# solislemuslab/BayesianNetworkRegression.jl

Hardware: AMD Instinct MI355X
Metric: Gibbs iterations/sec (all chains) (higher is better)
Workload: dtype f64; 1 GPU; synthetic n=500 V=100 (q=5050) R=7, 8 chains total, 8 per GPU; chains_total=8, chains_per_gpu=8, seed=20240501

## Files before the change

bayesiannetworkregression.jl_amd/csrc/bnr_kernels.h:

```cpp
#pragma once
#include "bnr_device.h"

#define BNR_RMAX 32
#define BNR_NB 32
#define BNR_GT 64


#define BNR_GLOBAL_PTR(member) d.member = (decltype(d.member))(__attribute__((address_space(1))) void *)(unsigned long long)(d.member)
__device__ __forceinline__ bnr_dev bnr_globalized(const bnr_dev *src)
{
    bnr_dev d = *src;
    BNR_GLOBAL_PTR(X); BNR_GLOBAL_PTR(X8); BNR_GLOBAL_PTR(XM); BNR_GLOBAL_PTR(Sdig); BNR_GLOBAL_PTR(y); BNR_GLOBAL_PTR(ek); BNR_GLOBAL_PTR(el); BNR_GLOBAL_PTR(trace); BNR_GLOBAL_PTR(plan);
    BNR_GLOBAL_PTR(pbase); BNR_GLOBAL_PTR(Wbuf); BNR_GLOBAL_PTR(sz); BNR_GLOBAL_PTR(PW); BNR_GLOBAL_PTR(PA); BNR_GLOBAL_PTR(PG);
    BNR_GLOBAL_PTR(Gpart); BNR_GLOBAL_PTR(E); BNR_GLOBAL_PTR(gmap); BNR_GLOBAL_PTR(a3); BNR_GLOBAL_PTR(xw); BNR_GLOBAL_PTR(a4);
    BNR_GLOBAL_PTR(res); BNR_GLOBAL_PTR(xg); BNR_GLOBAL_PTR(bw); BNR_GLOBAL_PTR(wv); BNR_GLOBAL_PTR(scal); BNR_GLOBAL_PTR(Minv);
    BNR_GLOBAL_PTR(Psum); BNR_GLOBAL_PTR(counters); BNR_GLOBAL_PTR(dbg); BNR_GLOBAL_PTR(stamp); BNR_GLOBAL_PTR(gprog); BNR_GLOBAL_PTR(gmapc); BNR_GLOBAL_PTR(dfctl);
    return d;
}
struct bnr_one {
    bnr_dev d;
    static constexpr bool whole = true, lone = true;
    __device__ __forceinline__ const bnr_dev &get() const { return d; }
    __device__ __forceinline__ const bnr_dev &get_x() const { return d; }
    __device__ __forceinline__ const bnr_dev &at(int) const { return d; }
// ... 902 lines not shown
    unsigned char *sX = (unsigned char *)smem_i8;
    bnr_i4 *sDig = (bnr_i4 *)(sX + 4 * BNR_I8_TB);
    const int tid = threadIdx.x, wave = tid >> 6, lane = tid & 63, ln = lane & 15, lq = lane >> 4;
    const int ng = cd.kcp / 16;
    for (int idx = tid; idx < L * ng; idx += 256) {
        const int l = idx / ng, g = idx % ng;
        sDig[idx] = *(const bnr_i4 *)(cd.Sdig + (size_t)l * cd.kslab + (size_t)ks * cd.kcp + 16 * g);
    }
    const int srow = tid >> 3, scol = tid & 7;
    const unsigned char *gI = cd.XM + (size_t)(ti * BNR_GT + srow) * cd.kslab + (size_t)ks * cd.kcp + 16 * scol;
    const unsigned char *gJ = cd.XM + (size_t)(tj * BNR_GT + srow) * cd.kslab + (size_t)ks * cd.kcp + 16 * scol;
    const size_t r32 = (size_t)32 * cd.kslab;
    const int soff = srow * BNR_I8_RS + 16 * scol;
    bnr_i4 r0 = {0, 0, 0, 0}, r1 = r0, r2 = r0, r3 = r0;
    const int nbatch = cd.kcp / 128, nb = nbatch + ((cd.kcp % 128) ? 1 : 0);
    auto load = [&](int b) {
        const int o = 128 * b;
        if (b < nbatch || scol < 4) { r0 = *(const bnr_i4 *)(gI + o); r1 = *(const bnr_i4 *)(gI + r32 + o); r2 = *(const bnr_i4 *)(gJ + o); r3 = *(const bnr_i4 *)(gJ + r32 + o); }
    };
    auto store = [&](int buf) {
        unsigned char *d = sX + buf * 2 * BNR_I8_TB + soff;
        *(bnr_i4 *)d = r0; *(bnr_i4 *)(d + 32 * BNR_I8_RS) = r1; *(bnr_i4 *)(d + BNR_I8_TB) = r2; *(bnr_i4 *)(d + BNR_I8_TB + 32 * BNR_I8_RS) = r3;
    };
    bnr_i4 acc[L][4];
#pragma unroll
    for (int l = 0; l < L; ++l)
#pragma unroll
        for (int a = 0; a < 4; ++a) acc[l][a] = bnr_i4{0, 0, 0, 0};
    load(0); store(0);
    if (nb > 1) load(1);
    __syncthreads();
    const int fa = ln * BNR_I8_RS + 16 * lq + BNR_I8_TB, fb = (wave * 16 + ln) * BNR_I8_RS + 16 * lq;
    for (int b = 0; b < nb; ++b) {
        const unsigned char *xb = sX + (b & 1) * 2 * BNR_I8_TB;
        const int nk = (b < nbatch) ? 2 : 1;
        bnr_i4 dgall;
        {
            const int pl = ln & 7, pk = ln >> 3, lcl = pl < L ? pl : L - 1;
            int gi = (2 * b + pk) * 4 + lq;
            gi = gi < ng ? gi : ng - 1;
            dgall = sDig[lcl * ng + gi];
        }
#pragma unroll
        for (int kk = 0; kk < 2; ++kk) {
            if (kk >= nk) break;
            const bnr_i4 a0 = *(const bnr_i4 *)(xb + fa + 64 * kk), a1 = *(const bnr_i4 *)(xb + fa + 16 * BNR_I8_RS + 64 * kk);
            const bnr_i4 a2 = *(const bnr_i4 *)(xb + fa + 32 * BNR_I8_RS + 64 * kk), a3 = *(const bnr_i4 *)(xb + fa + 48 * BNR_I8_RS + 64 * kk);
            const bnr_i4 b0 = *(const bnr_i4 *)(xb + fb + 64 * kk);
#pragma unroll
            for (int l = 0; l < L; ++l) {
                bnr_i4 m0;
                if (kk == 0) {
#pragma unroll
                    for (int d = 0; d < 4; ++d) m0[d] = b0[d] & bnr_row_bcast<0>(dgall[d], l);
                } else {
#pragma unroll
                    for (int d = 0; d < 4; ++d) m0[d] = b0[d] & bnr_row_bcast<8>(dgall[d], l);
                }
                acc[l][0] = __builtin_amdgcn_mfma_i32_16x16x64_i8(a0, m0, acc[l][0], 0, 0, 0);
                acc[l][1] = __builtin_amdgcn_mfma_i32_16x16x64_i8(a1, m0, acc[l][1], 0, 0, 0);
                acc[l][2] = __builtin_amdgcn_mfma_i32_16x16x64_i8(a2, m0, acc[l][2], 0, 0, 0);
                acc[l][3] = __builtin_amdgcn_mfma_i32_16x16x64_i8(a3, m0, acc[l][3], 0, 0, 0);
            }
            if (kk == 0 && b + 1 < nb) { store((b + 1) & 1); if (b + 2 < nb) load(b + 2); }
        }
        __syncthreads();
    }
    const double sc = -cd.scal[SC_I8SCALE];
    double *out = cd.Gpart + ((size_t)ks * ntl + t) * (BNR_GT * BNR_GT);
#pragma unroll
    for (int jt = 0; jt < 4; ++jt)
#pragma unroll
        for (int r = 0; r < 4; ++r) {
            double v = (double)acc[0][jt][r];
#pragma unroll
            for (int l = 1; l < L; ++l) v = v * 256.0 + (double)acc[l][jt][r];
            out[(jt * 16 + 4 * lq + r) * BNR_GT + wave * 16 + ln] = v * sc;
        }
}

__host__ __device__ inline int bnr_ldE(int n_pad) { return 2 * n_pad + BNR_NB; }

#define BNR_CRITICAL_PATH() __builtin_amdgcn_s_setprio(3)
template <class SRC>
__global__ __launch_bounds__(256) void k_gram_reduce(const SRC chain_src, int s)
{
    BNR_CRITICAL_PATH();
    const bnr_dev &cd = chain_src.get();
    int t = blockIdx.x, ti = 0;
    while ((ti + 1) * (ti + 2) / 2 <= t) ++ti;
    int tj = t - ti * (ti + 1) / 2;
    const int ntl = cd.ntile * (cd.ntile + 1) / 2;
    const size_t ld = bnr_ldE(cd.n_pad), tsz = BNR_GT * BNR_GT;
    const int idx = blockIdx.y * 512 + 2 * threadIdx.x;
    const double *src = cd.Gpart + (size_t)t * tsz + idx;
    bnr_d2 acc = {0.0, 0.0};
    int ks = 0;
    for (; ks + 3 < cd.ksplit; ks += 4) {
        bnr_d2 v0 = *(const bnr_d2 *)(src + (size_t)ks * ntl * tsz), v1 = *(const bnr_d2 *)(src + (size_t)(ks + 1) * ntl * tsz);
        bnr_d2 v2 = *(const bnr_d2 *)(src + (size_t)(ks + 2) * ntl * tsz), v3 = *(const bnr_d2 *)(src + (size_t)(ks + 3) * ntl * tsz);
        acc += v0; acc += v1; acc += v2; acc += v3;
    }
    for (; ks < cd.ksplit; ++ks) acc += *(const bnr_d2 *)(src + (size_t)ks * ntl * tsz);
    const int i = ti * BNR_GT + idx % BNR_GT, j = tj * BNR_GT + idx / BNR_GT;
    if (i == j) acc[0] += 1.0;
    if (i + 1 == j) acc[1] += 1.0;
    *(bnr_d2 *)(cd.E + (size_t)i + ld * j) = acc;
    const int nwg = gridDim.x * gridDim.y, wg = blockIdx.x * gridDim.y + blockIdx.y, np = cd.n_pad;
    for (size_t e = ((size_t)wg * 256 + threadIdx.x) * 2; e < (size_t)np * np; e += (size_t)nwg * 512) {
        int r = (int)(e % np), c = (int)(e / np);
        if (r / BNR_NB > c / BNR_NB) continue;
        bnr_d2 v = {(r == c) ? 1.0 : 0.0, (r + 1 == c) ? 1.0 : 0.0};
        *(bnr_d2 *)(cd.E + (size_t)(np + r) + ld * c) = v;
    }
    if (threadIdx.x == 0) cd.stamp[blockIdx.x * 8 + blockIdx.y] = cd.plan[cd.pbase[0] + s].it;
    if (blockIdx.x == 0 && blockIdx.y == 0 && (int)threadIdx.x <= cd.ntile) cd.gprog[threadIdx.x] = 0u;
}

__device__ __forceinline__ double bnr_readlane(double v, int srclane)
{
    int lo = __double2loint(v), hi = __double2hiint(v);
    lo = __builtin_amdgcn_readlane(lo, srclane);
    hi = __builtin_amdgcn_readlane(hi, srclane);
    return __hiloint2double(hi, lo);
}
#define BNR_LP (BNR_NB + 1)
__host__ __device__ inline int bnr_chol_npanel(int nbk, int p) { (void)p; return nbk + 1; }
__host__ __device__ inline int bnr_chol_ntile(int nbk, int p)
{
    if (p == 0) return 0;
    int m = nbk - (p + 1);
    return m * (m + 1) / 2 + m * p;
}
__host__ __device__ inline int bnr_chol_nsuper(int nbk, int p)
{
    if (p == 0) return 0;
    int ms = (nbk - (p + 1) + 1) / 2;
    return ms * (ms + 1) / 2 + ms * ((p + 1) / 2);
}

__device__ __forceinline__ bnr_d4 bnr_tile_update(const double *colrows, const double *rowrows, size_t ld, int lane, bnr_d4 c)
{
    const int ln = lane & 15, lk = lane >> 4;
    double av[8], bv[8];
#pragma unroll
    for (int ks = 0; ks < 8; ++ks) {
        av[ks] = colrows[(size_t)ln + ld * (size_t)(4 * ks + lk)];
        bv[ks] = rowrows[(size_t)ln + ld * (size_t)(4 * ks + lk)];
    }
#pragma unroll
    for (int ks = 0; ks < 8; ++ks) c = __builtin_amdgcn_mfma_f64_16x16x4f64(-av[ks], bv[ks], c, 0, 0, 0);
    return c;
}

#define BNR_L1S 80
#define BNR_PIPE_SPINS (1 << 16)
#define BNR_PIPE_SENT_HI 0x7FF8DEAD
__device__ __forceinline__ double bnr_canon_nan(double v) { return v == v ? v : __hiloint2double(0x7FF80000, 0); }
struct alignas(16) bnr_panelp_lds {
    double sD[BNR_NB * BNR_LP], sB[BNR_NB * BNR_LP];
    double sL[BNR_NB][64];
};
__device__ __forceinline__ unsigned bnr_lds_addr(const void *p) { return (unsigned)(unsigned long long)(__attribute__((address_space(3))) const void *)p; }
struct bnr_no_hook { __device__ __forceinline__ void operator()() const {} };
template <int N, int COFF, int PUB, class HOOK = bnr_no_hook>
__device__ __forceinline__ int bnr_sweepN(double (&a)[N], int lane, unsigned pub_addr, HOOK hook = HOOK())
{
    int bad = 0;
    double lprev = 0.0;
    double piv = bnr_readlane(a[0], COFF);
#pragma unroll
    for (int j = 0; j < N; ++j) {
        double tk[N];
        double s1 = 0.0, s2 = 0.0, s3 = 0.0;
        if (j + 1 < N) { s1 = bnr_readlane(a[j + 1], COFF + j + 1); s2 = bnr_readlane(a[j], COFF + j + 1); }
        if (j + 2 < N) s3 = bnr_readlane(a[j], COFF + j + 2);
        if (!(piv > 0.0)) bad = 1;
        double y = __builtin_amdgcn_rsq(piv);
        if (j == 0) hook();
        if (j >= 1) {
#pragma unroll
            for (int k = j + 2; k < N; ++k) tk[k] = bnr_readlane(lprev, COFF + k);
        }
        const double e = fma(-(piv * y), y, 1.0);
        const double rinv = fma(y * e, fma(0.375, e, 0.5), y);
        const double t1 = s2 * rinv;
        piv = fma(-t1, t1, s1);
        double lj = a[j] * rinv;
        a[j] = lj;
        if (PUB == 2) asm volatile("ds_write_b64 %1, %2 offset:%3" : "+v"(piv) : "v"(pub_addr), "v"(lj), "n"(512 * j) : "memory");
        if (j + 1 < N) a[j + 1] = fma(-lj, t1, a[j + 1]);
        if (j + 2 < N) a[j + 2] = fma(-lj, s3 * rinv, a[j + 2]);
        if (j >= 1) {
#pragma unroll
            for (int k = j + 2; k < N; ++k) a[k] = fma(-lprev, tk[k], a[k]);
        }
        lprev = lj;
    }
    return bad;
}
template <int COFF>
__device__ __forceinline__ int bnr_sweep16(double (&a)[16], int lane) { return bnr_sweepN<16, COFF, 0>(a, lane, 0u); }
template <int W>
__device__ __forceinline__ int bnr_pipe_wave(bnr_panelp_lds &sh, int lane, double *dst, size_t ld, unsigned long long *ph = nullptr)
{
#ifdef BNR_STAMPS
#define BNR_PPH(i) do { if (ph && lane == 0) ph[i] = __builtin_amdgcn_s_memtime(); } while (0)
#else
#define BNR_PPH(i) do { } while (0)
#endif
    constexpr int C0 = 8 * W;
    const int rr = lane & 31;
    const double *src = (lane < 32) ? sh.sD : sh.sB;
    double a[8];
#pragma unroll
    for (int c = 0; c < 8; ++c) a[c] = src[rr + BNR_LP * (C0 + c)];
    int bad = 0;
#define BNR_PIPE_HERE(X0, X1) __all(__double2hiint(X0) != BNR_PIPE_SENT_HI && __double2hiint(X1) != BNR_PIPE_SENT_HI)
    unsigned vc = bnr_lds_addr(&sh.sL[0][lane]), vm = bnr_lds_addr(&sh.sL[0][C0 + (lane & 7)]);
    double x0 = 0.0, x1 = 0.0, m0 = 0.0, m1 = 0.0, y0 = 0.0, y1 = 0.0, q0 = 0.0, q1 = 0.0;
#define BNR_DPP_READ4(X0, X1, M0, M1, OFF)                                                                                                                   \
    do { asm volatile("ds_read_b64 %0, %4 offset:%6\n\tds_read_b64 %1, %4 offset:%7\n\tds_read_b64 %2, %5 offset:%6\n\tds_read_b64 %3, %5 offset:%7"          \
                 : "=&v"(X0), "=&v"(X1), "=&v"(M0), "=&v"(M1) : "v"(vc), "v"(vm), "n"(OFF), "n"((OFF) + 512) : "memory");                                    \
         asm volatile("" : "+v"(a[0]), "+v"(a[1]), "+v"(a[2]), "+v"(a[3]), "+v"(a[4]), "+v"(a[5]), "+v"(a[6]), "+v"(a[7])); } while (0)
#define BNR_DPP_WAIT4(X0, X1, M0, M1) asm volatile("s_waitcnt lgkmcnt(0)" : "+v"(X0), "+v"(X1), "+v"(M0), "+v"(M1), "+v"(a[0]), "+v"(a[1]), "+v"(a[2]), "+v"(a[3]), "+v"(a[4]), "+v"(a[5]), "+v"(a[6]), "+v"(a[7]) :: "memory")
#define BNR_DPP_FMA(C, MM, X) asm("v_fmac_f64_dpp %0, -%1, %2 row_newbcast:%3 row_mask:0xf bank_mask:0xf" : "+v"(a[C]) : "v"(MM), "v"(X), "n"(C))
#define BNR_DPP_APPLY(CFROM, X0, X1, M0, M1)                                                                                                                 \
    do { _Pragma("unroll") for (int c_ = (CFROM); c_ < 8; ++c_) {                                                                                            \
             switch (c_) {                                                                                                                                   \
             case 0: BNR_DPP_FMA(0, M0, X0); BNR_DPP_FMA(0, M1, X1); break; case 1: BNR_DPP_FMA(1, M0, X0); BNR_DPP_FMA(1, M1, X1); break;                     \
             case 2: BNR_DPP_FMA(2, M0, X0); BNR_DPP_FMA(2, M1, X1); break; case 3: BNR_DPP_FMA(3, M0, X0); BNR_DPP_FMA(3, M1, X1); break;                     \
             case 4: BNR_DPP_FMA(4, M0, X0); BNR_DPP_FMA(4, M1, X1); break; case 5: BNR_DPP_FMA(5, M0, X0); BNR_DPP_FMA(5, M1, X1); break;                     \
             case 6: BNR_DPP_FMA(6, M0, X0); BNR_DPP_FMA(6, M1, X1); break; default: BNR_DPP_FMA(7, M0, X0); BNR_DPP_FMA(7, M1, X1); break; } } } while (0)
#define BNR_DPP_TRIP(X0, X1, M0, M1, OFF, Y0, Y1, Q0, Q1)                                                                \
    do {                                                                                                                \
        BNR_DPP_WAIT4(X0, X1, M0, M1);                                                                                  \
        if (!BNR_PIPE_HERE(X0, X1)) {                                                                                   \
            int spins = 0;                                                                                              \
            do {                                                                                                        \
                if (++spins > BNR_PIPE_SPINS) { bad = 1; break; }                                                       \
                BNR_DPP_READ4(X0, X1, M0, M1, OFF);                                                                     \
                BNR_DPP_WAIT4(X0, X1, M0, M1);                                                                          \
            } while (!BNR_PIPE_HERE(X0, X1));                                                                           \
        }                                                                                                               \
        BNR_DPP_READ4(Y0, Y1, Q0, Q1, (OFF) + 1024);                                                                    \
        BNR_DPP_APPLY(0, X0, X1, M0, M1);                                                                               \
    } while (0)
    if (W > 0) {
        constexpr int NT = C0 / 2;
        BNR_DPP_READ4(x0, x1, m0, m1, 0);
#pragma unroll 1
        for (int t = 0; t + 2 < NT; t += 2) {
            BNR_DPP_TRIP(x0, x1, m0, m1, 0, y0, y1, q0, q1);
            BNR_DPP_TRIP(y0, y1, q0, q1, 1024, x0, x1, m0, m1);
            vc += 2048; vm += 2048;
        }
        BNR_DPP_TRIP(x0, x1, m0, m1, 0, y0, y1, q0, q1);
        BNR_DPP_WAIT4(y0, y1, q0, q1);
        if (!BNR_PIPE_HERE(y0, y1)) {
            int spins = 0;
            do {
                if (++spins > BNR_PIPE_SPINS) { bad = 1; break; }
                BNR_DPP_READ4(y0, y1, q0, q1, 1024);
                BNR_DPP_WAIT4(y0, y1, q0, q1);
            } while (!BNR_PIPE_HERE(y0, y1));
        }
        BNR_DPP_FMA(0, q0, y0); BNR_DPP_FMA(0, q1, y1); BNR_DPP_FMA(1, q0, y0); BNR_DPP_FMA(1, q1, y1);
    }
    if (W == 1) BNR_PPH(3);
    if (W == 3) BNR_PPH(6);
    bad |= bnr_sweepN<8, C0, (W < 3 ? 2 : 0)>(a, lane, bnr_lds_addr(&sh.sL[C0][lane]), [&]() { if (W > 0) BNR_DPP_APPLY(2, y0, y1, q0, q1); });
    if (W == 0) BNR_PPH(2);
    if (W == 1) BNR_PPH(4);
    if (W == 2) BNR_PPH(5);
    if (W == 3) BNR_PPH(7);
    if (dst && lane >= 32) {
#pragma unroll
        for (int c = 0; c < 8; ++c) dst[(size_t)rr + ld * (size_t)(C0 + c)] = a[c];
    }
    return bad;
}
__device__ __forceinline__ int bnr_panel_sweep_pipe(bnr_panelp_lds &sh, const bnr_d4 &cD, const bnr_d4 &cB, int tid, double *dst, size_t ld, unsigned long long *ph = nullptr)
{
    const int wave = tid >> 6, lane = tid & 63, mt = wave >> 1, nt = wave & 1, ln = lane & 15, lq = lane >> 4;
#ifdef BNR_STAMPS
    if (ph && tid == 0) ph[0] = __builtin_amdgcn_s_memtime();
#endif
    {
        const double sent = __hiloint2double(BNR_PIPE_SENT_HI, 0);
        double *sl = &sh.sL[0][0];
#pragma unroll
        for (int i = 0; i < 6; ++i) sl[tid + 256 * i] = sent;
    }
#pragma unroll
    for (int r = 0; r < 4; ++r) {
        sh.sD[(nt * 16 + ln) + BNR_LP * (mt * 16 + lq + 4 * r)] = bnr_canon_nan(cD[r]);
        sh.sB[(nt * 16 + ln) + BNR_LP * (mt * 16 + lq + 4 * r)] = bnr_canon_nan(cB[r]);
    }
    __syncthreads();
#ifdef BNR_STAMPS
    if (ph && tid == 0) ph[1] = __builtin_amdgcn_s_memtime();
#endif
    if (wave == 0) return bnr_pipe_wave<0>(sh, lane, dst, ld, ph);
    if (wave == 1) return bnr_pipe_wave<1>(sh, lane, dst, ld, ph);
    if (wave == 2) return bnr_pipe_wave<2>(sh, lane, dst, ld, ph);
    return bnr_pipe_wave<3>(sh, lane, dst, ld, ph);
}
template <int NT>
__device__ __forceinline__ void bnr_gsum_frag(const bnr_dev &cd, int rho, int c, int at0, int bt0, int ln, int lq, bnr_d4 (&out)[NT][NT])
{
    const int ti = rho >> 1, tj = c >> 1, ntl = cd.ntile * (cd.ntile + 1) / 2;
    const size_t tsz = BNR_GT * BNR_GT, plane = (size_t)ntl * tsz;
    const double *src = cd.Gpart + (size_t)(ti * (ti + 1) / 2 + tj) * tsz + (size_t)((c & 1) * BNR_NB + 16 * at0 + lq) * BNR_GT + (rho & 1) * BNR_NB + 16 * bt0 + ln;
#pragma unroll
    for (int at = 0; at < NT; ++at)
#pragma unroll
        for (int bt = 0; bt < NT; ++bt) out[at][bt] = bnr_d4{0.0, 0.0, 0.0, 0.0};
    constexpr int KU = NT == 1 ? 8 : 4;
    const int klast = cd.ksplit - 1;
    for (int ks0 = 0; ks0 < cd.ksplit; ks0 += KU) {
        bnr_d4 v[KU][NT][NT];
#pragma unroll
        for (int u = 0; u < KU; ++u) {
            const size_t po = (size_t)(ks0 + u < klast ? ks0 + u : klast) * plane;
#pragma unroll
            for (int at = 0; at < NT; ++at)
#pragma unroll
                for (int bt = 0; bt < NT; ++bt)
#pragma unroll
                    for (int r = 0; r < 4; ++r) v[u][at][bt][r] = *(src + po + (size_t)(16 * at + 4 * r) * BNR_GT + 16 * bt);
        }
#pragma unroll
        for (int u = 0; u < KU; ++u) {
#pragma unroll
            for (int at = 0; at < NT; ++at)
#pragma unroll
                for (int bt = 0; bt < NT; ++bt)
#pragma unroll
                    for (int r = 0; r < 4; ++r) out[at][bt][r] += (ks0 + u <= klast) ? v[u][at][bt][r] : 0.0;
        }
    }
    if (rho == c) {
#pragma unroll
        for (int at = 0; at < NT; ++at)
#pragma unroll
            for (int bt = 0; bt < NT; ++bt)
#pragma unroll
                for (int r = 0; r < 4; ++r) if (16 * (bt0 + bt) + ln == 16 * (at0 + at) + lq + 4 * r) out[at][bt][r] += 1.0;
    }
}
template <int EPW>
__device__ __forceinline__ void bnr_reduce_parts(const bnr_dev &cd, int g0, int nwg, int wg, int s)
{
    constexpr int KB = EPW == 4 ? 4 : 8;
    const int tid = threadIdx.x, t = g0 >> 3, part0 = g0 & 7;
    const int ntl = cd.ntile * (cd.ntile + 1) / 2, ksplit = cd.ksplit;
    const size_t ld = (size_t)2 * cd.n_pad + BNR_NB, tsz = BNR_GT * BNR_GT, plane = (size_t)ntl * tsz;
    const double *src = cd.Gpart + (size_t)t * tsz + part0 * 512 + 2 * tid;
    bnr_d2 v[KB][EPW], acc[EPW];
    const int pb = *(const volatile int *)cd.pbase;
#define BNR_RP_LOAD(KS0)                                                                                                          \
    _Pragma("unroll") for (int u = 0; u < KB; ++u) {                                                                              \
        _Pragma("unroll") for (int e = 0; e < EPW; ++e) v[u][e] = bnr_d2{0.0, 0.0};                                               \
        if ((KS0) + u < ksplit) {                                                                                                 \
            _Pragma("unroll") for (int e = 0; e < EPW; ++e) v[u][e] = *(const bnr_d2 *)(src + (size_t)((KS0) + u) * plane + e * 512); \
        }                                                                                                                         \
    }
    BNR_RP_LOAD(0)
    const unsigned int it = cd.plan[pb + s].it;
    const int np = cd.n_pad;
    for (size_t e = ((size_t)wg * 256 + tid) * 2; e < (size_t)np * np; e += (size_t)nwg * 512) {
        const int r = (int)(e % np), c = (int)(e / np);
        if ((r < BNR_NB && c < BNR_NB) || r / BNR_NB > c / BNR_NB) continue;
        bnr_d2 y = {(r == c) ? 1.0 : 0.0, (r + 1 == c) ? 1.0 : 0.0};
        *(bnr_d2 *)(cd.E + (size_t)(np + r) + ld * c) = y;
    }
    if (wg == 0 && tid <= cd.ntile) cd.gprog[tid] = 0u;
#pragma unroll
    for (int e = 0; e < EPW; ++e) acc[e] = bnr_d2{0.0, 0.0};
    for (int ks0 = 0;;) {
#pragma unroll
        for (int u = 0; u < KB; ++u)
            if (ks0 + u < ksplit) {
#pragma unroll
                for (int e = 0; e < EPW; ++e) acc[e] += v[u][e];
            }
        ks0 += KB;
        if (ks0 >= ksplit) break;
        BNR_RP_LOAD(ks0)
    }
#undef BNR_RP_LOAD
    int ti = 0;
    while ((ti + 1) * (ti + 2) / 2 <= t) ++ti;
    const int tj = t - ti * (ti + 1) / 2;
#pragma unroll
    for (int e = 0; e < EPW; ++e) {
        const int idx = (part0 + e) * 512 + 2 * tid;
        const int i = ti * BNR_GT + idx % BNR_GT, j = tj * BNR_GT + idx / BNR_GT;
        if (i == j) acc[e][0] += 1.0;
        if (i + 1 == j) acc[e][1] += 1.0;
        if (j >= BNR_NB) *(bnr_d2 *)(cd.E + (size_t)i + ld * j) = acc[e];
    }
    if (tid < EPW) cd.stamp[g0 + tid] = it;
#ifdef BNR_STAMPS
    if (tid == 0) atomicMax((unsigned long long *)&cd.dbg[7], (unsigned long long)__builtin_amdgcn_s_memrealtime());
#endif
}
#define BNR_CHOL_WG_PER_CU 4
template <class SRC>
__global__ __launch_bounds__(256, BNR_CHOL_WG_PER_CU) void k_chol_step(const SRC chain_src, int p, int s, int tpw, int spw, int fuse0)
{
    BNR_CRITICAL_PATH();
#ifdef BNR_STAMPS
    const unsigned long long t_entry = __builtin_amdgcn_s_memtime();
#endif
    const bnr_dev &cd = chain_src.get_x();
    __shared__ bnr_panelp_lds sh;
    static_assert(sizeof(sh.sL) == 2 * BNR_NB * BNR_NB * sizeof(double), "the two fetched blocks of panel p - 1 live where the sweep's published columns will be");
    static_assert(BNR_CHOL_WG_PER_CU * sizeof(bnr_panelp_lds) <= 160 * 1024, "BNR_CHOL_WG_PER_CU workgroups must fit a CU's LDS");
    double (*sPO)[BNR_NB * BNR_NB] = (double (*)[BNR_NB * BNR_NB])&sh.sL[0][0];
    const int tid = threadIdx.x, wave = tid >> 6, lane = tid & 63, nbk = cd.n_pad / BNR_NB;
    const size_t ld = bnr_ldE(cd.n_pad);
    const int npanel = bnr_chol_npanel(nbk, p);
    const int pc = p * BNR_NB, kc = pc - BNR_NB;
    const int mt = wave >> 1, nt = wave & 1;
    const int ln = lane & 15, lq = lane >> 4;
    double *E = cd.E;
    if (SRC::whole && p == 0 && (int)blockIdx.y >= npanel) {
        const int wg = (int)blockIdx.y - npanel, nwg = (int)gridDim.y - npanel;
        if (SRC::lone || tpw == 1) bnr_reduce_parts<1>(cd, wg, nwg, wg, s);
        else if (tpw == 4) bnr_reduce_parts<4>(cd, 4 * wg, nwg, wg, s);
        else bnr_reduce_parts<2>(cd, 2 * wg, nwg, wg, s);
        return;
    }
    if ((int)blockIdx.y >= npanel) {
        const int m = nbk - (p + 1);
        if (tpw == 0) {
            const int ms = (m + 1) / 2, ntri = ms * (ms + 1) / 2, nsup = bnr_chol_nsuper(nbk, p);
            for (int u = 0; u < spw; ++u) {
                int t = ((int)blockIdx.y - npanel) * spw + u, R0, C0;
                if (t >= nsup) break;
                bool ident = false;
                if (t < ntri) {
                    int ti = 0;
                    while ((ti + 1) * (ti + 2) / 2 <= t) ++ti;
                    int tj = t - ti * (ti + 1) / 2;
                    R0 = p + 1 + 2 * ti; C0 = p + 1 + 2 * tj;
                } else {
                    t -= ntri;
                    const int ps = (p + 1) / 2;
                    C0 = p + 1 + 2 * (t / ps); R0 = nbk + 2 * (t % ps);
                    ident = true;
                }
                const int rho = R0 + (wave >> 1), j = C0 + (wave & 1);
                const bool ok = j < nbk && (ident ? (rho - nbk < p) : (rho < nbk && rho >= j));
                if (!ok) continue;
                double *cp = E + (size_t)(rho * BNR_NB + ln) + ld * (size_t)(j * BNR_NB + lq);
                bnr_d4 c[2][2];
#pragma unroll
                for (int a = 0; a < 2; ++a)
#pragma unroll
                    for (int b = 0; b < 2; ++b)
#pragma unroll
                        for (int r = 0; r < 4; ++r) c[a][b][r] = cp[(size_t)(16 * b) + ld * (size_t)(16 * a + 4 * r)];
                const double *colrows = E + (size_t)(j * BNR_NB) + ld * (size_t)kc, *rowrows = E + (size_t)(rho * BNR_NB) + ld * (size_t)kc;
                double av[2][8], bv[2][8];
#pragma unroll
                for (int ks = 0; ks < 8; ++ks) {
                    const size_t o = (size_t)ln + ld * (size_t)(4 * ks + lq);
                    av[0][ks] = colrows[o]; av[1][ks] = colrows[o + 16];
                    bv[0][ks] = rowrows[o]; bv[1][ks] = rowrows[o + 16];
                }
#pragma unroll
                for (int ks = 0; ks < 8; ++ks)
#pragma unroll
                    for (int a = 0; a < 2; ++a)
#pragma unroll
                        for (int b = 0; b < 2; ++b) c[a][b] = __builtin_amdgcn_mfma_f64_16x16x4f64(-av[a][ks], bv[b][ks], c[a][b], 0, 0, 0);
#pragma unroll
                for (int a = 0; a < 2; ++a)
#pragma unroll
                    for (int b = 0; b < 2; ++b)
#pragma unroll
                        for (int r = 0; r < 4; ++r) cp[(size_t)(16 * b) + ld * (size_t)(16 * a + 4 * r)] = c[a][b][r];
            }
#ifdef BNR_STAMPS
            if (tid == 0) atomicMax((unsigned long long *)&cd.dbg[p * 8 + 7], (unsigned long long)__builtin_amdgcn_s_memrealtime());
#endif
            return;
        }
        const int ntri = m * (m + 1) / 2, ntot = bnr_chol_ntile(nbk, p);
        const int t0 = ((int)blockIdx.y - npanel) * tpw;
        for (int tt = 0; tt < tpw && t0 + tt < ntot; ++tt) {
            int t = t0 + tt, rho, j;
            if (t < ntri) {
                int ti = 0;
                while ((ti + 1) * (ti + 2) / 2 <= t) ++ti;
                int tj = t - ti * (ti + 1) / 2;
                rho = p + 1 + ti; j = p + 1 + tj;
            } else {
                t -= ntri;
                j = p + 1 + t / p;
                rho = nbk + t % p;
            }
            double *cp = E + (size_t)(rho * BNR_NB + nt * 16 + ln) + ld * (size_t)(j * BNR_NB + mt * 16 + lq);
            bnr_d4 c;
#pragma unroll
            for (int r = 0; r < 4; ++r) c[r] = cp[ld * (size_t)(4 * r)];
            c = bnr_tile_update(E + (size_t)(j * BNR_NB + mt * 16) + ld * (size_t)kc, E + (size_t)(rho * BNR_NB + nt * 16) + ld * (size_t)kc, ld, lane, c);
#pragma unroll
            for (int r = 0; r < 4; ++r) cp[ld * (size_t)(4 * r)] = c[r];
        }
#ifdef BNR_STAMPS
        if (tid == 0) atomicMax((unsigned long long *)&cd.dbg[p * 8 + 7], (unsigned long long)__builtin_amdgcn_s_memrealtime());
#endif
        return;
    }
    const int b = blockIdx.y;
    if (p == (fuse0 ? 1 : 0) && b == 0) {
        const unsigned int it = cd.plan[cd.pbase[0] + s].it;
        const int nred = 8 * (cd.ntile * (cd.ntile + 1) / 2);
        for (int w = tid; w < nred; w += blockDim.x)
            if (cd.stamp[w] != it) atomicAdd((unsigned long long *)&cd.counters[8], 1ull);
    }
#ifdef BNR_STAMPS
#define BNR_STAMP(slot) do { if (b == 0 && tid == 0) cd.dbg[p * 8 + (slot)] = __builtin_amdgcn_s_memtime(); } while (0)
#else
#define BNR_STAMP(slot) do { } while (0)
#endif
    BNR_STAMP(0);
#ifdef BNR_STAMPS
    if (tid == 0) {
        const unsigned long long rt = __builtin_amdgcn_s_memrealtime();
        if (b == 0) cd.dbg[p * 8 + 1] = rt;
        atomicMax((unsigned long long *)&cd.dbg[p * 8 + 6], rt);
    }
#endif
    int rho;
    if (b < nbk - p) rho = p + b;
    else rho = nbk + (b - (nbk - p));
    bnr_d4 cD, cB;
    if (p == 0 && fuse0) {
        bnr_d4 t1[1][1];
        bnr_gsum_frag<1>(cd, 0, 0, mt, nt, ln, lq, t1);
        cD = t1[0][0];
        if (rho < nbk) { bnr_gsum_frag<1>(cd, rho, 0, mt, nt, ln, lq, t1); cB = t1[0][0]; }
        else {
#pragma unroll
            for (int r = 0; r < 4; ++r) cB[r] = (nt * 16 + ln == mt * 16 + lq + 4 * r) ? 1.0 : 0.0;
        }
    } else {
        const double *dp = E + (size_t)(pc + nt * 16 + ln) + ld * (size_t)(pc + mt * 16 + lq);
        const double *bp = E + (size_t)(rho * BNR_NB + nt * 16 + ln) + ld * (size_t)(pc + mt * 16 + lq);
#pragma unroll
        for (int r = 0; r < 4; ++r) { cD[r] = dp[ld * (size_t)(4 * r)]; cB[r] = bp[ld * (size_t)(4 * r)]; }
#ifdef BNR_STAMPS
        if (b == 0 && tid == 0 && p < 24) cd.dbg[3800 + 4 * p] = t_entry;
#endif
        if (p > 0) {
            const int fc = tid >> 4, fr = (tid & 15) * 2;
            const double *gP = E + (size_t)(pc + fr) + ld * (size_t)(kc + fc), *gO = E + (size_t)(rho * BNR_NB + fr) + ld * (size_t)(kc + fc);
            const bnr_d2 p0 = *(const bnr_d2 *)gP, p1 = *(const bnr_d2 *)(gP + ld * 16), o0 = *(const bnr_d2 *)gO, o1 = *(const bnr_d2 *)(gO + ld * 16);
            const int wo = (fr ^ ((fc & 1) << 4)) + 32 * fc;
            *(bnr_d2 *)&sPO[0][wo] = p0; *(bnr_d2 *)&sPO[0][wo + 512] = p1;
            *(bnr_d2 *)&sPO[1][wo] = o0; *(bnr_d2 *)&sPO[1][wo + 512] = o1;
            __syncthreads();
#ifdef BNR_STAMPS
            if (b == 0 && tid == 0 && p < 24) cd.dbg[3800 + 4 * p + 1] = __builtin_amdgcn_s_memtime();
#endif
            const int lk = lane >> 4;
            double av[8], b1[8], b2[8];
#pragma unroll
            for (int ks = 0; ks < 8; ++ks) {
                const int c = 4 * ks + lk, sw = (c & 1) << 4;
                av[ks] = sPO[0][((mt * 16 + ln) ^ sw) + 32 * c]; b1[ks] = sPO[0][((nt * 16 + ln) ^ sw) + 32 * c]; b2[ks] = sPO[1][((nt * 16 + ln) ^ sw) + 32 * c];
            }
            __syncthreads();
#pragma unroll
            for (int ks = 0; ks < 8; ++ks) cD = __builtin_amdgcn_mfma_f64_16x16x4f64(-av[ks], b1[ks], cD, 0, 0, 0);
#pragma unroll
            for (int ks = 0; ks < 8; ++ks) cB = __builtin_amdgcn_mfma_f64_16x16x4f64(-av[ks], b2[ks], cB, 0, 0, 0);
#ifdef BNR_STAMPS
            { double chk = cD[3] + cB[3]; asm volatile("" :: "v"(chk)); if (b == 0 && tid == 0 && p < 24) cd.dbg[3800 + 4 * p + 2] = __builtin_amdgcn_s_memtime(); }
#endif
        }
    }
    BNR_STAMP(2);
    double *dst = rho != p ? E + (size_t)(rho * BNR_NB) + ld * (size_t)pc : nullptr;
#ifdef BNR_STAMPS
    const int bad = bnr_panel_sweep_pipe(sh, cD, cB, tid, dst, ld, b == 0 ? cd.dbg + 128 + p * 8 : nullptr);
#else
    const int bad = bnr_panel_sweep_pipe(sh, cD, cB, tid, dst, ld);
#endif
    if (bad && lane == 0) bnr_flag_gfail(cd);
    BNR_STAMP(3);
    BNR_STAMP(4);
#ifdef BNR_STAMPS
    if (lane == 0) atomicMax((unsigned long long *)&cd.dbg[p * 8 + 5], (unsigned long long)__builtin_amdgcn_s_memrealtime());
    if (b == 0 && tid == 192 && p < 48) { cd.dbg[3900 + 2 * p] = __builtin_amdgcn_s_memrealtime(); cd.dbg[3901 + 2 * p] = __builtin_amdgcn_s_memtime(); }
#endif
}

struct bnr_panel2_lds {
    double sDaa[BNR_NB * BNR_LP], sDba[BNR_NB * BNR_LP], sDbb[BNR_NB * BNR_LP], sOa[BNR_NB * BNR_LP], sOb[BNR_NB * BNR_LP];
    double pad_[2][2][BNR_NB];
    double sL1[2][16 * BNR_L1S];
};
__device__ __forceinline__ void bnr_panel_load16(double (&a)[16], const double *sD, const double *sB, int lane, int c0)
{
    const double *src = (lane < 32) ? sD : sB;
    const int rr = lane & 31;
#pragma unroll
    for (int c = 0; c < 16; ++c) a[c] = src[rr + BNR_LP * (c0 + c)];
}
__device__ __forceinline__ void bnr_lds_tile_update(double *sC, const double *colside, const double *rowside, int mt, int nt, int ln, int lq)
{
    bnr_d4 c;
#pragma unroll
    for (int r = 0; r < 4; ++r) c[r] = sC[(nt * 16 + ln) + BNR_LP * (mt * 16 + lq + 4 * r)];
#pragma unroll
    for (int ks = 0; ks < 8; ++ks)
        c = __builtin_amdgcn_mfma_f64_16x16x4f64(-colside[(mt * 16 + ln) + BNR_LP * (4 * ks + lq)], rowside[(nt * 16 + ln) + BNR_LP * (4 * ks + lq)], c, 0, 0, 0);
#pragma unroll
    for (int r = 0; r < 4; ++r) sC[(nt * 16 + ln) + BNR_LP * (mt * 16 + lq + 4 * r)] = c[r];
}
__device__ __forceinline__ void bnr_mid_tile(double *sX, int rowb, const double *sL1, int lrow, int ln, int lq)
{
    bnr_d4 c;
#pragma unroll
    for (int r = 0; r < 4; ++r) c[r] = sX[(rowb + ln) + BNR_LP * (16 + lq + 4 * r)];
#pragma unroll
    for (int ks = 0; ks < 4; ++ks) {
        const double av = sL1[(4 * ks + lq) * BNR_L1S + 16 + ln];
        const double bv = sL1[(4 * ks + lq) * BNR_L1S + lrow + ln];
        c = __builtin_amdgcn_mfma_f64_16x16x4f64(-av, bv, c, 0, 0, 0);
    }
#pragma unroll
    for (int r = 0; r < 4; ++r) sX[(rowb + ln) + BNR_LP * (16 + lq + 4 * r)] = c[r];
}
__host__ __device__ inline int bnr_chol2_nsuper(int nbk, int P, int lazy = 0)
{
    if (P == 0) return 0;
    const int m = nbk - 2 * P - 2, ms = (m + 1) / 2;
    if (m <= 0) return 0;
    if (lazy && !(P & 1)) return ms + P;
    return ms * (ms + 1) / 2 + ms * P;
}
template <int NQ>
__device__ __forceinline__ void bnr_super_update(double *E, size_t ld, int rho, int j, int q0, int ln, int lq)
{
    double *cp = E + (size_t)(rho * BNR_NB + ln) + ld * (size_t)(j * BNR_NB + lq);
    bnr_d4 c[2][2];
#pragma unroll
    for (int at = 0; at < 2; ++at)
#pragma unroll
        for (int bt = 0; bt < 2; ++bt)
#pragma unroll
            for (int r = 0; r < 4; ++r) c[at][bt][r] = cp[(size_t)(16 * bt) + ld * (size_t)(16 * at + 4 * r)];
    double av[NQ][2][8], bv[NQ][2][8];
#pragma unroll
    for (int qq = 0; qq < NQ; ++qq) {
        const int kc = (q0 + qq) * BNR_NB;
        const double *colrows = E + (size_t)(j * BNR_NB) + ld * (size_t)kc, *rowrows = E + (size_t)(rho * BNR_NB) + ld * (size_t)kc;
#pragma unroll
        for (int ks = 0; ks < 8; ++ks) {
            const size_t o = (size_t)ln + ld * (size_t)(4 * ks + lq);
            av[qq][0][ks] = colrows[o]; av[qq][1][ks] = colrows[o + 16];
            bv[qq][0][ks] = rowrows[o]; bv[qq][1][ks] = rowrows[o + 16];
        }
    }
#pragma unroll
    for (int qq = 0; qq < NQ; ++qq)
#pragma unroll
        for (int ks = 0; ks < 8; ++ks)
#pragma unroll
            for (int at = 0; at < 2; ++at)
#pragma unroll
                for (int bt = 0; bt < 2; ++bt) c[at][bt] = __builtin_amdgcn_mfma_f64_16x16x4f64(-av[qq][at][ks], bv[qq][bt][ks], c[at][bt], 0, 0, 0);
#pragma unroll
    for (int at = 0; at < 2; ++at)
#pragma unroll
        for (int bt = 0; bt < 2; ++bt)
#pragma unroll
            for (int r = 0; r < 4; ++r) cp[(size_t)(16 * bt) + ld * (size_t)(16 * at + 4 * r)] = c[at][bt][r];
}
template <class SRC>
__global__ __launch_bounds__(256, 1) void k_chol_step2(const SRC chain_src, int P, int s, int spw, int lazy)
{
    BNR_CRITICAL_PATH();
    const bnr_dev &cd = chain_src.get_x();
    __shared__ bnr_panel2_lds sh;
    const int tid = threadIdx.x, wave = tid >> 6, lane = tid & 63, nbk = cd.n_pad / BNR_NB;
    const size_t ld = bnr_ldE(cd.n_pad);
    const int a = 2 * P, b = a + 1, pa = a * BNR_NB, pb = b * BNR_NB;
    const int ln = lane & 15, lq = lane >> 4;
    double *E = cd.E;
    if ((int)blockIdx.y >= nbk) {
        const int m = nbk - 2 * P - 2, ms = (m + 1) / 2, nsup = bnr_chol2_nsuper(nbk, P, lazy);
        const bool near = lazy && !(P & 1);
        const int ntri = near ? ms : ms * (ms + 1) / 2;
        const int q0 = (lazy && (P & 1) && a >= 4) ? a - 4 : a - 2, nq = a - q0;
        for (int u = 0; u < spw; ++u) {
            int t = ((int)blockIdx.y - nbk) * spw + u, R0, C0;
            if (t >= nsup) break;
            bool ident = false;
            if (t < ntri) {
                int ti = 0, tj = 0;
                if (near) ti = t;
                else {
                    while ((ti + 1) * (ti + 2) / 2 <= t) ++ti;
                    tj = t - ti * (ti + 1) / 2;
                }
                R0 = a + 2 + 2 * ti; C0 = a + 2 + 2 * tj;
            } else {
                t -= ntri;
                C0 = a + 2 + 2 * (t / P); R0 = nbk + 2 * (t % P);
                ident = true;
            }
            const int rho = R0 + (wave >> 1), j = C0 + (wave & 1);
            const bool ok = j < nbk && (ident ? (rho - nbk < a) : (rho < nbk && rho >= j));
            if (!ok) continue;
            if (nq == 4) bnr_super_update<4>(E, ld, rho, j, q0, ln, lq);
            else bnr_super_update<2>(E, ld, rho, j, q0, ln, lq);
        }
        return;
    }
    const int bi = blockIdx.y;
    if (P == 0 && bi == 0) {
        const unsigned int it = cd.plan[cd.pbase[0] + s].it;
        const int nred = 8 * (cd.ntile * (cd.ntile + 1) / 2);
        for (int w = tid; w < nred; w += blockDim.x)
            if (cd.stamp[w] != it) atomicAdd((unsigned long long *)&cd.counters[8], 1ull);
    }
    const int nmat = nbk - b - 1;
    const int R = bi < nmat ? b + 1 + bi : nbk + (bi - nmat);
    const bool only_b = bi >= nmat && (bi - nmat) == b;
    {
        const int mt = wave >> 1, nt = wave & 1;
// ... 1206 lines not shown
```

Baseline: 23020 iterations/s.

## Generate identity-augmented Cholesky blocks on the fly instead of prefilling E

Drops the grid-wide loop in the reduce phase that wrote an identity/zero pattern into the augmented right-hand-side region of E. The panel and trailing-update kernels now synthesize those blocks when they are first touched, by zero-masking loaded values with a register-opaque keep mask and injecting ones on the diagonal. This removes a full n_pad^2 store pass from the critical path, at the cost of extra branching and mask logic in the panel kernels. It also risks correctness if any consumer reads those blocks before the generating step.

```diff
diff --git a/bayesiannetworkregression.jl_amd/csrc/bnr_kernels.h b/bayesiannetworkregression.jl_amd/csrc/bnr_kernels.h
--- a/bayesiannetworkregression.jl_amd/csrc/bnr_kernels.h
+++ b/bayesiannetworkregression.jl_amd/csrc/bnr_kernels.h
@@ -1078,6 +1078,22 @@
     for (int ks = 0; ks < 8; ++ks) c = __builtin_amdgcn_mfma_f64_16x16x4f64(-av[ks], bv[ks], c, 0, 0, 0);
     return c;
 }
+__device__ __forceinline__ bnr_d4 bnr_tile_update_keep(const double *colrows, const double *rowrows, size_t ld, int lane, bnr_d4 c, unsigned int keep)
+{
+    const int ln = lane & 15, lk = lane >> 4;
+    double av[8], bv[8];
+#pragma unroll
+    for (int ks = 0; ks < 8; ++ks) {
+        av[ks] = colrows[(size_t)ln + ld * (size_t)(4 * ks + lk)];
+        bv[ks] = rowrows[(size_t)ln + ld * (size_t)(4 * ks + lk)];
+    }
+    __builtin_amdgcn_sched_barrier(0);
+#pragma unroll
+    for (int r = 0; r < 4; ++r) c[r] = __hiloint2double((int)(__double2hiint(c[r]) & keep), (int)(__double2loint(c[r]) & keep));
+#pragma unroll
+    for (int ks = 0; ks < 8; ++ks) c = __builtin_amdgcn_mfma_f64_16x16x4f64(-av[ks], bv[ks], c, 0, 0, 0);
+    return c;
+}
 
 #define BNR_L1S 80
 #define BNR_PIPE_SPINS (1 << 16)
@@ -1276,7 +1292,7 @@
     }
 }
 template <int EPW>
-__device__ __forceinline__ void bnr_reduce_parts(const bnr_dev &cd, int g0, int nwg, int wg, int s)
+__device__ __forceinline__ void bnr_reduce_parts(const bnr_dev &cd, int g0, int wg, int s)
 {
     constexpr int KB = EPW == 4 ? 4 : 8;
     const int tid = threadIdx.x, t = g0 >> 3, part0 = g0 & 7;
@@ -1294,13 +1310,6 @@
     }
     BNR_RP_LOAD(0)
     const unsigned int it = cd.plan[pb + s].it;
-    const int np = cd.n_pad;
-    for (size_t e = ((size_t)wg * 256 + tid) * 2; e < (size_t)np * np; e += (size_t)nwg * 512) {
-        const int r = (int)(e % np), c = (int)(e / np);
-        if ((r < BNR_NB && c < BNR_NB) || r / BNR_NB > c / BNR_NB) continue;
-        bnr_d2 y = {(r == c) ? 1.0 : 0.0, (r + 1 == c) ? 1.0 : 0.0};
-        *(bnr_d2 *)(cd.E + (size_t)(np + r) + ld * c) = y;
-    }
     if (wg == 0 && tid <= cd.ntile) cd.gprog[tid] = 0u;
 #pragma unroll
     for (int e = 0; e < EPW; ++e) acc[e] = bnr_d2{0.0, 0.0};
@@ -1353,10 +1362,10 @@
     const int ln = lane & 15, lq = lane >> 4;
     double *E = cd.E;
     if (SRC::whole && p == 0 && (int)blockIdx.y >= npanel) {
-        const int wg = (int)blockIdx.y - npanel, nwg = (int)gridDim.y - npanel;
-        if (SRC::lone || tpw == 1) bnr_reduce_parts<1>(cd, wg, nwg, wg, s);
-        else if (tpw == 4) bnr_reduce_parts<4>(cd, 4 * wg, nwg, wg, s);
-        else bnr_reduce_parts<2>(cd, 2 * wg, nwg, wg, s);
+        const int wg = (int)blockIdx.y - npanel;
+        if (SRC::lone || tpw == 1) bnr_reduce_parts<1>(cd, wg, wg, s);
+        else if (tpw == 4) bnr_reduce_parts<4>(cd, 4 * wg, wg, s);
+        else bnr_reduce_parts<2>(cd, 2 * wg, wg, s);
         return;
     }
     if ((int)blockIdx.y >= npanel) {
@@ -1383,12 +1392,19 @@
                 if (!ok) continue;
                 double *cp = E + (size_t)(rho * BNR_NB + ln) + ld * (size_t)(j * BNR_NB + lq);
                 bnr_d4 c[2][2];
+                const bool first = ident && rho - nbk == p - 1;
 #pragma unroll
                 for (int a = 0; a < 2; ++a)
 #pragma unroll
-                    for (int b = 0; b < 2; ++b)
-#pragma unroll
-                        for (int r = 0; r < 4; ++r) c[a][b][r] = cp[(size_t)(16 * b) + ld * (size_t)(16 * a + 4 * r)];
+                    for (int b = 0; b < 2; ++b) c[a][b] = bnr_d4{0.0, 0.0, 0.0, 0.0};
+                if (!first) {
+#pragma unroll
+                    for (int a = 0; a < 2; ++a)
+#pragma unroll
+                        for (int b = 0; b < 2; ++b)
+#pragma unroll
+                            for (int r = 0; r < 4; ++r) c[a][b][r] = cp[(size_t)(16 * b) + ld * (size_t)(16 * a + 4 * r)];
+                }
                 const double *colrows = E + (size_t)(j * BNR_NB) + ld * (size_t)kc, *rowrows = E + (size_t)(rho * BNR_NB) + ld * (size_t)kc;
                 double av[2][8], bv[2][8];
 #pragma unroll
@@ -1419,6 +1435,7 @@
         const int t0 = ((int)blockIdx.y - npanel) * tpw;
         for (int tt = 0; tt < tpw && t0 + tt < ntot; ++tt) {
             int t = t0 + tt, rho, j;
+            bool first = false;
             if (t < ntri) {
                 int ti = 0;
                 while ((ti + 1) * (ti + 2) / 2 <= t) ++ti;
@@ -1428,12 +1445,16 @@
                 t -= ntri;
                 j = p + 1 + t / p;
                 rho = nbk + t % p;
+                first = t % p == p - 1;
             }
             double *cp = E + (size_t)(rho * BNR_NB + nt * 16 + ln) + ld * (size_t)(j * BNR_NB + mt * 16 + lq);
+            const double *lp = first ? E + (size_t)(rho * BNR_NB + nt * 16 + ln) + ld * (size_t)(kc + mt * 16 + lq) : cp;
+            unsigned int keep = first ? 0u : ~0u;
+            asm volatile("" : "+v"(keep));
             bnr_d4 c;
 #pragma unroll
-            for (int r = 0; r < 4; ++r) c[r] = cp[ld * (size_t)(4 * r)];
-            c = bnr_tile_update(E + (size_t)(j * BNR_NB + mt * 16) + ld * (size_t)kc, E + (size_t)(rho * BNR_NB + nt * 16) + ld * (size_t)kc, ld, lane, c);
+            for (int r = 0; r < 4; ++r) c[r] = lp[ld * (size_t)(4 * r)];
+            c = bnr_tile_update_keep(E + (size_t)(j * BNR_NB + mt * 16) + ld * (size_t)kc, E + (size_t)(rho * BNR_NB + nt * 16) + ld * (size_t)kc, ld, lane, c, keep);
 #pragma unroll
             for (int r = 0; r < 4; ++r) cp[ld * (size_t)(4 * r)] = c[r];
         }
@@ -1477,16 +1498,33 @@
         }
     } else {
         const double *dp = E + (size_t)(pc + nt * 16 + ln) + ld * (size_t)(pc + mt * 16 + lq);
-        const double *bp = E + (size_t)(rho * BNR_NB + nt * 16 + ln) + ld * (size_t)(pc + mt * 16 + lq);
-#pragma unroll
-        for (int r = 0; r < 4; ++r) { cD[r] = dp[ld * (size_t)(4 * r)]; cB[r] = bp[ld * (size_t)(4 * r)]; }
+        const bool ynew = rho == nbk + p, yfirst = p > 0 && rho == nbk + p - 1, ygen = ynew || yfirst;
+        const double *bp = ygen ? dp : E + (size_t)(rho * BNR_NB + nt * 16 + ln) + ld * (size_t)(pc + mt * 16 + lq);
+        unsigned int keepB = ygen ? 0u : ~0u, keepO = ynew ? 0u : ~0u;
+        asm volatile("" : "+v"(keepB), "+v"(keepO));
+#pragma unroll
+        for (int r = 0; r < 4; ++r) {
+            cD[r] = dp[ld * (size_t)(4 * r)];
+            cB[r] = bp[ld * (size_t)(4 * r)];
+        }
+#define BNR_YGEN_CB()                                                                                                                           \
+        _Pragma("unroll") for (int r = 0; r < 4; ++r) {                                                                                         \
+            const unsigned int one = (ynew && nt * 16 + ln == mt * 16 + lq + 4 * r) ? 0x3ff00000u : 0u;               \
+            cB[r] = __hiloint2double((int)((__double2hiint(cB[r]) & keepB) | one), (int)(__double2loint(cB[r]) & keepB));                       \
+        }
 #ifdef BNR_STAMPS
         if (b == 0 && tid == 0 && p < 24) cd.dbg[3800 + 4 * p] = t_entry;
 #endif
         if (p > 0) {
             const int fc = tid >> 4, fr = (tid & 15) * 2;
-            const double *gP = E + (size_t)(pc + fr) + ld * (size_t)(kc + fc), *gO = E + (size_t)(rho * BNR_NB + fr) + ld * (size_t)(kc + fc);
-            const bnr_d2 p0 = *(const bnr_d2 *)gP, p1 = *(const bnr_d2 *)(gP + ld * 16), o0 = *(const bnr_d2 *)gO, o1 = *(const bnr_d2 *)(gO + ld * 16);
+            const double *gP = E + (size_t)(pc + fr) + ld * (size_t)(kc + fc), *gO = ynew ? gP : E + (size_t)(rho * BNR_NB + fr) + ld * (size_t)(kc + fc);
+            const bnr_d2 p0 = *(const bnr_d2 *)gP, p1 = *(const bnr_d2 *)(gP + ld * 16);
+            bnr_d2 o0 = *(const bnr_d2 *)gO, o1 = *(const bnr_d2 *)(gO + ld * 16);
+#pragma unroll
+            for (int e = 0; e < 2; ++e) {
+                o0[e] = __hiloint2double((int)(__double2hiint(o0[e]) & keepO), (int)(__double2loint(o0[e]) & keepO));
+                o1[e] = __hiloint2double((int)(__double2hiint(o1[e]) & keepO), (int)(__double2loint(o1[e]) & keepO));
+            }
             const int wo = (fr ^ ((fc & 1) << 4)) + 32 * fc;
             *(bnr_d2 *)&sPO[0][wo] = p0; *(bnr_d2 *)&sPO[0][wo + 512] = p1;
             *(bnr_d2 *)&sPO[1][wo] = o0; *(bnr_d2 *)&sPO[1][wo + 512] = o1;
@@ -1502,6 +1540,7 @@
                 av[ks] = sPO[0][((mt * 16 + ln) ^ sw) + 32 * c]; b1[ks] = sPO[0][((nt * 16 + ln) ^ sw) + 32 * c]; b2[ks] = sPO[1][((nt * 16 + ln) ^ sw) + 32 * c];
             }
             __syncthreads();
+            BNR_YGEN_CB()
 #pragma unroll
             for (int ks = 0; ks < 8; ++ks) cD = __builtin_amdgcn_mfma_f64_16x16x4f64(-av[ks], b1[ks], cD, 0, 0, 0);
 #pragma unroll
@@ -1509,7 +1548,11 @@
 #ifdef BNR_STAMPS
             { double chk = cD[3] + cB[3]; asm volatile("" :: "v"(chk)); if (b == 0 && tid == 0 && p < 24) cd.dbg[3800 + 4 * p + 2] = __builtin_amdgcn_s_memtime(); }
 #endif
-        }
+        } else if (ynew) {
+#pragma unroll
+            for (int r = 0; r < 4; ++r) cB[r] = (nt * 16 + ln == mt * 16 + lq + 4 * r) ? 1.0 : 0.0;
+        }
+#undef BNR_YGEN_CB
     }
     BNR_STAMP(2);
     double *dst = rho != p ? E + (size_t)(rho * BNR_NB) + ld * (size_t)pc : nullptr;
```

After: 23020 iterations/s (median of 2 runs). About the same (-0.0%).
